# david8862/tf-keras-deeplabv3p-model-set

Hardware: AMD Instinct MI355X
Metric: images/sec (513x513, 21-class) MobileNetV2-DeepLabV3+ OS=16 training step (higher is better)
Workload: dtype f32

## Files before the change

tf-keras-deeplabv3p-model-set_amd/csrc/dwconv.hip:

```cpp
#include "bf16.h"
#include <stdlib.h>
#include <type_traits>

struct DwParams {
  const float* x; int ldx;
  const float* scale; const float* shift; int act;
  const float* w;
  float* y; int ldy;
  const float* dy; int lddy;
  float* partials;
  int N, H, W, C, Ho, Wo, stride, rate, pad_t, pad_l;
  int c4s, px, nslab, nbx, spr, th, nbands, ks, ks5;
  int uh;
  long long total;
  int flip, accumulate;
  int nt;
  int fast_rows;
  int tw;
  int lat;
  int bf16_io;
  const float* bb_z; int bb_ldz;
  const float* bb_scale; const float* bb_shift; const float* bb_mean; const float* bb_invstd; int bb_act;
  const float* fa_z; int fa_ldz;
  const float* fa_scale; const float* fa_shift; const float* fa_mean; const float* fa_invstd; const float* fa_coef; int fa_act;
  float* fa_dz; int fa_lddz;
  const float* up_x; int up_ld, up_h, up_w, up_C;
};

struct DwLerp { int lo, hi; float t; };
__device__ __forceinline__ DwLerp dw_lerp(int o, float scale, int in_size) {
  const float src = ((float)o + 0.5f) * scale - 0.5f;
  const float fl = floorf(src);
  DwLerp r;
  r.lo = max((int)fl, 0);
  r.hi = min((int)ceilf(src), in_size - 1);
  r.t = src - fl;
  return r;
}
__device__ __forceinline__ float4 dw_up_load(const float* img, int up_w, int up_ld, DwLerp ly, DwLerp lx) {
  const float4 tl = ld4(img + ((size_t)ly.lo * up_w + lx.lo) * up_ld);
  const float4 tr = ld4(img + ((size_t)ly.lo * up_w + lx.hi) * up_ld);
  const float4 bl = ld4(img + ((size_t)ly.hi * up_w + lx.lo) * up_ld);
  const float4 br = ld4(img + ((size_t)ly.hi * up_w + lx.hi) * up_ld);
  float4 o;
#define DW_LERP2(f) { const float top = tl.f + (tr.f - tl.f) * lx.t; const float bot = bl.f + (br.f - bl.f) * lx.t; o.f = top + (bot - top) * ly.t; }
  DW_LERP2(x) DW_LERP2(y) DW_LERP2(z) DW_LERP2(w)
#undef DW_LERP2
  return o;
}

__device__ __forceinline__ void bnb_accumulate(float4 (&s1)[2], float4 g, float4 zv, float4 bsc, float4 bsh, float4 bmu,
                                               float4 bis, int act) {
  const float4 u = fma4(zv, bsc, bsh);
  const float4 d = make_float4(g.x * act_grad(u.x, act), g.y * act_grad(u.y, act), g.z * act_grad(u.z, act),
                               g.w * act_grad(u.w, act));
  const float4 xh = make_float4((zv.x - bmu.x) * bis.x, (zv.y - bmu.y) * bis.y, (zv.z - bmu.z) * bis.z, (zv.w - bmu.w) * bis.w);
  s1[0] = add4(s1[0], d);
  s1[1] = fma4(d, xh, s1[1]);
}

template <int PRO>
__device__ __forceinline__ float4 prologue4(float4 v, float4 sc, float4 sh, int act) {
  if (PRO == 0) return v;
  v = fma4(v, sc, sh);
  if (PRO == 2) v = act_apply4(v, act);
  return v;
}

template <int KS, int TW, int S, int PRO, bool BNB = false, bool UP = false>
__global__ __launch_bounds__(256) void dw_fwd_seg(DwParams p) {
  constexpr int SEG = (TW - 1) * S + KS;
  const int b = blockIdx.x;
  const int slab = b / p.nbx;
  const int bx = b - slab * p.nbx;
  const int t = threadIdx.x;
  const int pl = t / p.c4s;
  const int cl = t - pl * p.c4s;
  const bool active = pl < p.px;
  const int cbase4 = slab * p.c4s;
  const int c = (cbase4 + cl) * 4;
  float4 s1[2] = {zero4(), zero4()};
  constexpr bool WLDS = KS == 5;
  extern __shared__ __attribute__((aligned(16))) float4 dw_w_lds[];
  if (WLDS) {
    for (int i = t; i < KS * KS * p.c4s; i += 256) {
      const int tap = i / p.c4s, lane = i - tap * p.c4s;
      dw_w_lds[i] = ld4(p.w + (size_t)(p.flip ? KS * KS - 1 - tap : tap) * p.C + (cbase4 + lane) * 4);
    }
    __syncthreads();
  }
  if (active) {
    float4 wreg[WLDS ? 1 : KS * KS];
    if (!WLDS) {
#pragma unroll
      for (int i = 0; i < KS * KS; ++i) wreg[i] = ld4(p.w + (size_t)(p.flip ? KS * KS - 1 - i : i) * p.C + c);
    }
    auto wtap = [&](int i) { return WLDS ? dw_w_lds[i * p.c4s + cl] : wreg[WLDS ? 0 : i]; };
    float4 sc = make_float4(1.f, 1.f, 1.f, 1.f), sh = zero4();
    if (p.scale) { sc = ld4(p.scale + c); sh = ld4(p.shift + c); }
    float4 bsc = zero4(), bsh = zero4(), bmu = zero4(), bis = zero4();
    if (BNB) { bsc = ld4(p.bb_scale + c); bsh = ld4(p.bb_shift + c); bmu = ld4(p.bb_mean + c); bis = ld4(p.bb_invstd + c); }
    const int act = p.act;
    const int th = p.th, nbands = p.nbands, rate = p.rate;
    XcdRange r = xcd_range(p.total, bx, p.nbx, p.px, pl);
    for (int s = r.begin; s < r.end; s += r.step) {
      const int strip = s % p.spr;
      int t2 = s / p.spr;
      const int band = t2 % nbands;
      t2 /= nbands;
      const int phase = t2 % (rate * rate);
      const int n = t2 / (rate * rate);
      const int py = phase / rate, pxo = phase - py * rate;
      const int u0 = strip * TW;
      const int v0 = band * p.uh / nbands, v1 = (band + 1) * p.uh / nbands;
      const int ox0 = pxo + u0 * rate;
      const int ix0 = ox0 * S - p.pad_l;
      const float* ximg = p.x + (size_t)n * p.H * p.W * p.ldx + c;
      int coff[SEG];
      bool cok[SEG];
#pragma unroll
      for (int i = 0; i < SEG; ++i) {
        const int ix = ix0 + i * rate;
        cok[i] = ix >= 0 && ix < p.W;
        coff[i] = ix * p.ldx;
      }
      DwLerp lxs[UP ? SEG : 1];
      const bool upl = UP && c < p.up_C;
      const float* uimg = nullptr;
      float usy = 0.f;
      if (UP) {
        const float usx = (float)p.up_w / (float)p.W;
        usy = (float)p.up_h / (float)p.H;
#pragma unroll
        for (int i = 0; i < SEG; ++i) lxs[i] = dw_lerp(min(max(ix0 + i * rate, 0), p.W - 1), usx, p.up_w);
        uimg = p.up_x + (size_t)n * p.up_h * p.up_w * p.up_ld + (upl ? c : 0);
      }
      float4 win[KS][SEG];
      float4 raw[S][SEG];
      {
        const int oy = py + v0 * rate;
#pragma unroll
        for (int ky = 0; ky < KS; ++ky) {
          const int iy = oy * S - p.pad_t + ky * rate;
          const bool yok = iy >= 0 && iy < p.H;
          const float* xrow = ximg + (size_t)iy * p.W * p.ldx;
#pragma unroll
          for (int i = 0; i < SEG; ++i) {
            win[ky][i] = zero4();
            if (yok && cok[i]) win[ky][i] = (UP && upl) ? dw_up_load(uimg, p.up_w, p.up_ld, dw_lerp(iy, usy, p.up_h), lxs[UP ? i : 0]) : ld4(xrow + coff[i]);
          }
        }
#pragma unroll
        for (int ky = 0; ky < KS; ++ky) {
          const int iy = oy * S - p.pad_t + ky * rate;
          const bool yok = iy >= 0 && iy < p.H;
#pragma unroll
          for (int i = 0; i < SEG; ++i) {
            const float4 a = prologue4<PRO>(win[ky][i], sc, sh, act);
            win[ky][i] = (yok && cok[i]) ? a : zero4();
          }
        }
      }
      const int vmax = (p.Ho - py + rate - 1) / rate;
      const int vend = v1 < vmax ? v1 : vmax;
      int coffc[SEG];
#pragma unroll
      for (int i = 0; i < SEG; ++i) coffc[i] = min(max(ix0 + i * rate, 0), p.W - 1) * p.ldx;
      auto row = [&](int v, auto fast_c, auto load_c) __attribute__((always_inline)) {
        constexpr bool FAST = decltype(fast_c)::value, LOAD = decltype(load_c)::value;
        const int oy = py + v * rate;
        const bool more = LOAD;
        float4 zv[TW];
        if (BNB) {
          const float* zrow = p.bb_z + (((size_t)n * p.Ho + oy) * p.Wo + ox0) * p.bb_ldz + c;
#pragma unroll
          for (int tw = 0; tw < TW; ++tw) zv[tw] = ld4(zrow + (size_t)min(tw * rate, p.Wo - 1 - ox0) * p.bb_ldz);
        }
        bool nyok[S];
#pragma unroll
        for (int q = 0; q < S; ++q) {
          const int iy = (oy + rate) * S - p.pad_t + (KS - S + q) * rate;
          nyok[q] = more && iy >= 0 && iy < p.H;
          if (FAST) {
            if (LOAD) {
              const float* xrow = ximg + (size_t)min(max(iy, 0), p.H - 1) * p.W * p.ldx;
#pragma unroll
              for (int i = 0; i < SEG; ++i) raw[q][i] = ld4(xrow + coffc[i]);
            }
          } else {
            const float* xrow = ximg + (size_t)iy * p.W * p.ldx;
#pragma unroll
            for (int i = 0; i < SEG; ++i) {
              raw[q][i] = zero4();
              if (nyok[q] && cok[i]) raw[q][i] = (UP && upl) ? dw_up_load(uimg, p.up_w, p.up_ld, dw_lerp(iy, usy, p.up_h), lxs[UP ? i : 0]) : ld4(xrow + coff[i]);
            }
          }
        }
        if (FAST) __builtin_amdgcn_sched_barrier(0);
        float4 acc[TW];
#pragma unroll
        for (int i = 0; i < TW; ++i) acc[i] = zero4();
        if (WLDS) asm volatile("" ::: "memory");
#pragma unroll
        for (int ky = 0; ky < KS; ++ky)
#pragma unroll
          for (int kx = 0; kx < KS; ++kx) {
            const float4 wv = wtap(ky * KS + kx);
#pragma unroll
            for (int tw = 0; tw < TW; ++tw) acc[tw] = fma4(win[ky][tw * S + kx], wv, acc[tw]);
          }
        float* yrow = p.y + (((size_t)n * p.Ho + oy) * p.Wo + ox0) * p.ldy + c;
#pragma unroll
        for (int tw = 0; tw < TW; ++tw) {
          if (FAST || ox0 + tw * rate < p.Wo) {
            float4 vv = acc[tw];
            float* yp = yrow + (size_t)tw * rate * p.ldy;
            if (!FAST && p.accumulate) vv = add4(vv, ld4(yp));
            if (FAST) { if (PRO != 0) st4_nt(yp, vv); else st4(yp, vv); }
            else if (p.nt) st4_nt(yp, vv); else st4(yp, vv);
            if (BNB) {
              bnb_accumulate(s1, vv, zv[tw], bsc, bsh, bmu, bis, p.bb_act);
            } else {
              s1[0] = add4(s1[0], vv);
              s1[1] = fma4(vv, vv, s1[1]);
            }
          }
        }
        if (!LOAD) return;
        if (FAST) __builtin_amdgcn_sched_barrier(0);
#pragma unroll
        for (int ky = 0; ky + S < KS; ++ky)
#pragma unroll
          for (int i = 0; i < SEG; ++i) win[ky][i] = win[ky + S][i];
#pragma unroll
        for (int q = 0; q < S; ++q)
#pragma unroll
          for (int i = 0; i < SEG; ++i) {
            float4 a = prologue4<PRO>(raw[q][i], sc, sh, act);
            if (FAST) asm volatile("" : "+v"(a.x), "+v"(a.y), "+v"(a.z), "+v"(a.w));
            win[KS - S + q][i] = (nyok[q] && cok[i]) ? a : zero4();
          }
      };
      constexpr bool HAS_FAST = PRO != 0 && !BNB && !UP;
      const bool fast = HAS_FAST && !p.accumulate && p.fast_rows && p.nt && ox0 + (TW - 1) * rate < p.Wo;
      if (HAS_FAST && fast) {
        for (int v = v0; v + 1 < vend; ++v) row(v, std::true_type{}, std::true_type{});
        if (vend > v0) row(vend - 1, std::true_type{}, std::false_type{});
      } else {
        for (int v = v0; v + 1 < vend; ++v) row(v, std::false_type{}, std::true_type{});
        if (vend > v0) row(vend - 1, std::false_type{}, std::false_type{});
      }
    }
  }
  if (p.partials) block_reduce_store<2>(s1, active, pl, cl, p.c4s, p.px, cbase4, p.C, p.partials + (size_t)bx * 2 * p.C);
}

__device__ __forceinline__ void pin4(float4& v) {
  asm volatile("" : "+v"(v.x), "+v"(v.y), "+v"(v.z), "+v"(v.w) : : "memory");
}

template <int TW, int PRO>
__global__ __launch_bounds__(256, 2) void dw5_rows(DwParams p) {
  constexpr int KS = 5, SEG = TW + KS - 1;
  const int b = blockIdx.x;
  const int slab = b / p.nbx;
  const int bx = b - slab * p.nbx;
  const int t = threadIdx.x;
  const int pl = t / p.c4s;
  const int cl = t - pl * p.c4s;
  const bool active = pl < p.px;
  const int cbase4 = slab * p.c4s;
  const int c = (cbase4 + cl) * 4;
  float4 s1[2] = {zero4(), zero4()};
  extern __shared__ __attribute__((aligned(16))) float4 dw_w_lds[];
  for (int i = t; i < KS * KS * p.c4s; i += 256) {
    const int tap = i / p.c4s, lane = i - tap * p.c4s;
    dw_w_lds[i] = ld4(p.w + (size_t)(p.flip ? KS * KS - 1 - tap : tap) * p.C + (cbase4 + lane) * 4);
  }
  __syncthreads();
  if (active) {
    float4 sc = make_float4(1.f, 1.f, 1.f, 1.f), sh = zero4();
    if (p.scale) { sc = ld4(p.scale + c); sh = ld4(p.shift + c); }
    const int act = p.act;
    const int th = p.th, nbands = p.nbands, rate = p.rate;
    const float4* wl = dw_w_lds + cl;
    const int c4s = p.c4s;
    XcdRange r = xcd_range(p.total, bx, p.nbx, p.px, pl);
    for (int s = r.begin; s < r.end; s += r.step) {
      const int strip = s % p.spr;
      int t2 = s / p.spr;
      const int band = t2 % nbands;
      t2 /= nbands;
      const int phase = t2 % (rate * rate);
      const int n = t2 / (rate * rate);
      const int py = phase / rate, pxo = phase - py * rate;
      const int v0 = band * p.uh / nbands, v1 = (band + 1) * p.uh / nbands;
      const int oy0 = py + v0 * rate;
      if (oy0 >= p.Ho) continue;
      int nv = (p.Ho - oy0 + rate - 1) / rate;
      if (nv > v1 - v0) nv = v1 - v0;
      const int ox0 = pxo + strip * TW * rate;
      const int ix0 = ox0 - p.pad_l;
      const float* ximg = p.x + (size_t)n * p.H * p.W * p.ldx + c;
      int coff[SEG];
      bool cok[SEG];
#pragma unroll
      for (int i = 0; i < SEG; ++i) {
        const int ix = ix0 + i * rate;
        cok[i] = ix >= 0 && ix < p.W;
        coff[i] = ix * p.ldx;
      }
      const int iy0 = oy0 - p.pad_t;
      const int nj = nv + KS - 1;
      float4 acc[KS][TW];
#pragma unroll
      for (int q = 0; q < KS; ++q)
#pragma unroll
        for (int tw = 0; tw < TW; ++tw) acc[q][tw] = zero4();
      float4 a[SEG];
      {
        const bool yok = iy0 >= 0 && iy0 < p.H;
        const float* xrow = ximg + (size_t)iy0 * p.W * p.ldx;
#pragma unroll
        for (int i = 0; i < SEG; ++i) {
          a[i] = zero4();
          if (yok && cok[i]) a[i] = ld4(xrow + coff[i]);
        }
#pragma unroll
        for (int i = 0; i < SEG; ++i) {
          const float4 v = prologue4<PRO>(a[i], sc, sh, act);
          a[i] = (yok && cok[i]) ? v : zero4();
        }
      }
      for (int j = 0; j < nj; ++j) {
        float4 nxt[SEG];
        const int iyn = iy0 + (j + 1) * rate;
        const bool nyok = j + 1 < nj && iyn >= 0 && iyn < p.H;
        {
          const float* xrow = ximg + (size_t)iyn * p.W * p.ldx;
#pragma unroll
          for (int i = 0; i < SEG; ++i) {
            nxt[i] = zero4();
            if (nyok && cok[i]) nxt[i] = ld4(xrow + coff[i]);
          }
        }
        const int vdone = j - (KS - 1);
        const int oyd = oy0 + vdone * rate;
        asm volatile("" ::: "memory");
        float4 wrow[2][KS];
#pragma unroll
        for (int kx = 0; kx < KS; ++kx) wrow[0][kx] = wl[kx * c4s];
#pragma unroll
        for (int ky = 0; ky < KS; ++ky) {
          if (ky + 1 < KS) {
#pragma unroll
            for (int kx = 0; kx < KS; ++kx) wrow[(ky + 1) & 1][kx] = wl[((ky + 1) * KS + kx) * c4s];
          }
#pragma unroll
          for (int kx = 0; kx < KS; ++kx) {
#pragma unroll
            for (int tw = 0; tw < TW; ++tw)
              acc[KS - 1 - ky][tw] = fma4(a[tw + kx], wrow[ky & 1][kx], acc[KS - 1 - ky][tw]);
          }
#pragma unroll
          for (int tw = 0; tw < TW; ++tw) pin4(acc[KS - 1 - ky][tw]);
        }
        if (vdone >= 0) {
          float* yrow = p.y + (((size_t)n * p.Ho + oyd) * p.Wo + ox0) * p.ldy + c;
#pragma unroll
          for (int tw = 0; tw < TW; ++tw) {
            if (ox0 + tw * rate < p.Wo) {
              float4 vv = acc[0][tw];
              float* yp = yrow + (size_t)tw * rate * p.ldy;
              if (p.accumulate) vv = add4(vv, ld4(yp));
              if (p.nt) st4_nt(yp, vv); else st4(yp, vv);
              s1[0] = add4(s1[0], vv);
              s1[1] = fma4(vv, vv, s1[1]);
            }
          }
        }
#pragma unroll
        for (int q = 0; q + 1 < KS; ++q)
#pragma unroll
          for (int tw = 0; tw < TW; ++tw) acc[q][tw] = acc[q + 1][tw];
#pragma unroll
        for (int tw = 0; tw < TW; ++tw) acc[KS - 1][tw] = zero4();
#pragma unroll
        for (int i = 0; i < SEG; ++i) {
          const float4 v = prologue4<PRO>(nxt[i], sc, sh, act);
          a[i] = (nyok && cok[i]) ? v : zero4();
        }
      }
    }
  }
  if (p.partials) block_reduce_store<2>(s1, active, pl, cl, p.c4s, p.px, cbase4, p.C, p.partials + (size_t)bx * 2 * p.C);
}

template <int TW, int PRO>
__global__ __launch_bounds__(256, 2) void dw5_wgrad_rows(DwParams p) {
  constexpr int KS = 5, SEG = TW + KS - 1;
  const int b = blockIdx.x;
  const int slab = b / p.nbx;
  const int bx = b - slab * p.nbx;
  const int t = threadIdx.x;
  const int pl = t / p.c4s;
  const int cl = t - pl * p.c4s;
  const bool active = pl < p.px;
  const int cbase4 = slab * p.c4s;
  const int c = (cbase4 + cl) * 4;
  float4 wacc[KS * KS];
#pragma unroll
  for (int i = 0; i < KS * KS; ++i) wacc[i] = zero4();
  if (active) {
    float4 sc = make_float4(1.f, 1.f, 1.f, 1.f), sh = zero4();
    if (p.scale) { sc = ld4(p.scale + c); sh = ld4(p.shift + c); }
    const int act = p.act;
    const int nbands = p.nbands, rate = p.rate;
    XcdRange r = xcd_range(p.total, bx, p.nbx, p.px, pl);
    for (int s = r.begin; s < r.end; s += r.step) {
      const int strip = s % p.spr;
      int t2 = s / p.spr;
      const int band = t2 % nbands;
      t2 /= nbands;
      const int phase = t2 % (rate * rate);
      const int n = t2 / (rate * rate);
      const int py = phase / rate, pxo = phase - py * rate;
      const int v0 = band * p.uh / nbands, v1 = (band + 1) * p.uh / nbands;
      const int oy0 = py + v0 * rate;
      if (oy0 >= p.Ho) continue;
      int nv = (p.Ho - oy0 + rate - 1) / rate;
      if (nv > v1 - v0) nv = v1 - v0;
      const int ox0 = pxo + strip * TW * rate;
      const int ix0 = ox0 - p.pad_l;
      const float* ximg = p.x + (size_t)n * p.H * p.W * p.ldx + c;
      const float* dimg = p.dy + ((size_t)n * p.Ho * p.Wo + ox0) * p.lddy + c;
      int coff[SEG];
      bool cok[SEG];
#pragma unroll
      for (int i = 0; i < SEG; ++i) {
        const int ix = ix0 + i * rate;
        cok[i] = ix >= 0 && ix < p.W;
        coff[i] = ix * p.ldx;
      }
      bool dok[TW];
#pragma unroll
      for (int tw = 0; tw < TW; ++tw) dok[tw] = ox0 + tw * rate < p.Wo;
      const int iy0 = oy0 - p.pad_t;
      const int nj = nv + KS - 1;
      float4 a[SEG];
      float4 dyw[KS][TW];
#pragma unroll
      for (int d = 0; d < KS; ++d)
#pragma unroll
        for (int tw = 0; tw < TW; ++tw) dyw[d][tw] = zero4();
      {
        const bool yok = iy0 >= 0 && iy0 < p.H;
        const float* xrow = ximg + (size_t)iy0 * p.W * p.ldx;
#pragma unroll
        for (int i = 0; i < SEG; ++i) {
          a[i] = zero4();
          if (yok && cok[i]) a[i] = ld4(xrow + coff[i]);
        }
        const float* drow = dimg + (size_t)oy0 * p.Wo * p.lddy;
#pragma unroll
        for (int tw = 0; tw < TW; ++tw)
          if (dok[tw]) dyw[KS - 1][tw] = ld4(drow + (size_t)tw * rate * p.lddy);
#pragma unroll
        for (int i = 0; i < SEG; ++i) {
          const float4 v = prologue4<PRO>(a[i], sc, sh, act);
          a[i] = (yok && cok[i]) ? v : zero4();
        }
      }
      for (int j = 0; j < nj; ++j) {
        float4 nxt[SEG], dyn[TW];
        const int iyn = iy0 + (j + 1) * rate;
        const bool nyok = j + 1 < nj && iyn >= 0 && iyn < p.H;
        const bool dyok = j + 1 < nv;
        {
          const float* xrow = ximg + (size_t)iyn * p.W * p.ldx;
#pragma unroll
          for (int i = 0; i < SEG; ++i) {
            nxt[i] = zero4();
            if (nyok && cok[i]) nxt[i] = ld4(xrow + coff[i]);
          }
          const float* drow = dimg + (size_t)(oy0 + (j + 1) * rate) * p.Wo * p.lddy;
#pragma unroll
          for (int tw = 0; tw < TW; ++tw) {
            dyn[tw] = zero4();
            if (dyok && dok[tw]) dyn[tw] = ld4(drow + (size_t)tw * rate * p.lddy);
          }
        }
#pragma unroll
        for (int ky = 0; ky < KS; ++ky)
#pragma unroll
          for (int kx = 0; kx < KS; ++kx)
#pragma unroll
            for (int tw = 0; tw < TW; ++tw)
              wacc[ky * KS + kx] = fma4(a[tw + kx], dyw[KS - 1 - ky][tw], wacc[ky * KS + kx]);
#pragma unroll
        for (int d = 0; d + 1 < KS; ++d)
#pragma unroll
          for (int tw = 0; tw < TW; ++tw) dyw[d][tw] = dyw[d + 1][tw];
#pragma unroll
        for (int tw = 0; tw < TW; ++tw) dyw[KS - 1][tw] = dyn[tw];
#pragma unroll
        for (int i = 0; i < SEG; ++i) {
          const float4 v = prologue4<PRO>(nxt[i], sc, sh, act);
          a[i] = (nyok && cok[i]) ? v : zero4();
        }
      }
    }
  }
  block_reduce_store<KS * KS>(wacc, active, pl, cl, p.c4s, p.px, cbase4, p.C,
                              p.partials + (size_t)bx * KS * KS * p.C);
}

template <int KS, int TW, int S, int PRO, bool BNA = false, bool UP = false>
__global__ __launch_bounds__(256) void dw_bwd_weight_seg(DwParams p) {
  constexpr int SEG = (TW - 1) * S + KS;
  const int b = blockIdx.x;
  const int slab = b / p.nbx;
  const int bx = b - slab * p.nbx;
  const int t = threadIdx.x;
  const int pl = t / p.c4s;
  const int cl = t - pl * p.c4s;
  const bool active = pl < p.px;
  const int cbase4 = slab * p.c4s;
  const int c = (cbase4 + cl) * 4;
  float4 wacc[KS * KS];
#pragma unroll
  for (int i = 0; i < KS * KS; ++i) wacc[i] = zero4();
  if (active) {
    float4 sc = make_float4(1.f, 1.f, 1.f, 1.f), sh = zero4();
    if (p.scale) { sc = ld4(p.scale + c); sh = ld4(p.shift + c); }
    const int act = p.act;
    const int th = p.th, nbands = p.nbands, rate = p.rate;
    float4 bA = zero4(), bC = zero4(), bD = zero4(), bsc = make_float4(1.f, 1.f, 1.f, 1.f), bsh = zero4();
    if (BNA) {
      if (p.fa_scale) { bsc = ld4(p.fa_scale + c); bsh = ld4(p.fa_shift + c); }
      const float4 mu = ld4(p.fa_mean + c), is = ld4(p.fa_invstd + c);
      const float4 c0 = ld4(p.fa_coef + c), c1 = ld4(p.fa_coef + p.C + c), c2 = ld4(p.fa_coef + 2 * p.C + c);
      bA = c0;
      bC = mul4(mul4(c0, is), c2);
      bD = make_float4(bC.x * mu.x - c0.x * c1.x, bC.y * mu.y - c0.y * c1.y, bC.z * mu.z - c0.z * c1.z, bC.w * mu.w - c0.w * c1.w);
    }
    XcdRange r = xcd_range(p.total, bx, p.nbx, p.px, pl);
    for (int s = r.begin; s < r.end; s += r.step) {
      const int strip = s % p.spr;
      int t2 = s / p.spr;
      const int band = t2 % nbands;
      t2 /= nbands;
      const int phase = t2 % (rate * rate);
      const int n = t2 / (rate * rate);
      const int py = phase / rate, pxo = phase - py * rate;
      const int u0 = strip * TW;
      const int v0 = band * p.uh / nbands, v1 = (band + 1) * p.uh / nbands;
      const int ox0 = pxo + u0 * rate;
      const int ix0 = ox0 * S - p.pad_l;
      const float* ximg = p.x + (size_t)n * p.H * p.W * p.ldx + c;
      int coff[SEG];
      bool cok[SEG];
#pragma unroll
      for (int i = 0; i < SEG; ++i) {
        const int ix = ix0 + i * rate;
        cok[i] = ix >= 0 && ix < p.W;
        coff[i] = ix * p.ldx;
      }
      DwLerp lxs[UP ? SEG : 1];
      const bool upl = UP && c < p.up_C;
      const float* uimg = nullptr;
      float usy = 0.f;
      if (UP) {
        const float usx = (float)p.up_w / (float)p.W;
        usy = (float)p.up_h / (float)p.H;
#pragma unroll
        for (int i = 0; i < SEG; ++i) lxs[i] = dw_lerp(min(max(ix0 + i * rate, 0), p.W - 1), usx, p.up_w);
        uimg = p.up_x + (size_t)n * p.up_h * p.up_w * p.up_ld + (upl ? c : 0);
      }
      float4 win[KS][SEG];
      float4 raw[S][SEG];
      {
        const int oy = py + v0 * rate;
#pragma unroll
        for (int ky = 0; ky < KS; ++ky) {
          const int iy = oy * S - p.pad_t + ky * rate;
          const bool yok = iy >= 0 && iy < p.H;
          const float* xrow = ximg + (size_t)iy * p.W * p.ldx;
#pragma unroll
          for (int i = 0; i < SEG; ++i) {
            win[ky][i] = zero4();
            if (yok && cok[i]) win[ky][i] = (UP && upl) ? dw_up_load(uimg, p.up_w, p.up_ld, dw_lerp(iy, usy, p.up_h), lxs[UP ? i : 0]) : ld4(xrow + coff[i]);
          }
        }
#pragma unroll
        for (int ky = 0; ky < KS; ++ky) {
          const int iy = oy * S - p.pad_t + ky * rate;
          const bool yok = iy >= 0 && iy < p.H;
#pragma unroll
          for (int i = 0; i < SEG; ++i) {
            const float4 a = prologue4<PRO>(win[ky][i], sc, sh, act);
            win[ky][i] = (yok && cok[i]) ? a : zero4();
          }
        }
      }
      for (int v = v0; v < v1; ++v) {
        const int oy = py + v * rate;
        if (oy >= p.Ho) break;
        const bool more = v + 1 < v1 && oy + rate < p.Ho;
        bool nyok[S];
#pragma unroll
        for (int q = 0; q < S; ++q) {
          const int iy = (oy + rate) * S - p.pad_t + (KS - S + q) * rate;
          nyok[q] = more && iy >= 0 && iy < p.H;
          const float* xrow = ximg + (size_t)iy * p.W * p.ldx;
#pragma unroll
          for (int i = 0; i < SEG; ++i) {
            raw[q][i] = zero4();
            if (nyok[q] && cok[i]) raw[q][i] = (UP && upl) ? dw_up_load(uimg, p.up_w, p.up_ld, dw_lerp(iy, usy, p.up_h), lxs[UP ? i : 0]) : ld4(xrow + coff[i]);
          }
        }
        float4 dyv[TW];
        const float* drow = p.dy + (((size_t)n * p.Ho + oy) * p.Wo + ox0) * p.lddy + c;
#pragma unroll
        for (int tw = 0; tw < TW; ++tw) {
          dyv[tw] = zero4();
          if (ox0 + tw * rate < p.Wo) dyv[tw] = ld4(drow + (size_t)tw * rate * p.lddy);
        }
        if (BNA) {
          const size_t pix = ((size_t)n * p.Ho + oy) * p.Wo + ox0;
          const float* zrow = p.fa_z + pix * p.fa_ldz + c;
          float4 zv[TW];
#pragma unroll
          for (int tw = 0; tw < TW; ++tw) {
            zv[tw] = zero4();
            if (ox0 + tw * rate < p.Wo) zv[tw] = ld4(zrow + (size_t)tw * rate * p.fa_ldz);
          }
          const int fact = p.fa_act;
#pragma unroll
          for (int tw = 0; tw < TW; ++tw) {
            const float4 z = zv[tw], g = dyv[tw];
            const float4 u = fma4(z, bsc, bsh);
            const float4 v = make_float4(fmaf(bA.x, g.x * act_grad(u.x, fact), fmaf(-bC.x, z.x, bD.x)),
                                         fmaf(bA.y, g.y * act_grad(u.y, fact), fmaf(-bC.y, z.y, bD.y)),
                                         fmaf(bA.z, g.z * act_grad(u.z, fact), fmaf(-bC.z, z.z, bD.z)),
                                         fmaf(bA.w, g.w * act_grad(u.w, fact), fmaf(-bC.w, z.w, bD.w)));
            const bool ok = ox0 + tw * rate < p.Wo;
            if (ok && p.fa_dz) st4(p.fa_dz + (pix + (size_t)tw * rate) * p.fa_lddz + c, v);
            dyv[tw] = ok ? v : zero4();
          }
        }
#pragma unroll
        for (int ky = 0; ky < KS; ++ky)
#pragma unroll
          for (int kx = 0; kx < KS; ++kx)
#pragma unroll
            for (int tw = 0; tw < TW; ++tw) wacc[ky * KS + kx] = fma4(win[ky][tw * S + kx], dyv[tw], wacc[ky * KS + kx]);
#pragma unroll
        for (int ky = 0; ky + S < KS; ++ky)
#pragma unroll
          for (int i = 0; i < SEG; ++i) win[ky][i] = win[ky + S][i];
#pragma unroll
        for (int q = 0; q < S; ++q)
#pragma unroll
          for (int i = 0; i < SEG; ++i) {
            const float4 a = prologue4<PRO>(raw[q][i], sc, sh, act);
            win[KS - S + q][i] = (nyok[q] && cok[i]) ? a : zero4();
          }
      }
    }
  }
  block_reduce_store<KS * KS>(wacc, active, pl, cl, p.c4s, p.px, cbase4, p.C,
// ... 402 lines not shown
  const int pl = t / p.c4s;
  const int cl = t - pl * p.c4s;
  const bool active = pl < p.px;
  const int cbase4 = slab * p.c4s;
  const int c = (cbase4 + cl) * 4;
  float4 wacc[KS * KS];
#pragma unroll
  for (int i = 0; i < KS * KS; ++i) wacc[i] = zero4();
  if (active) {
    float4 sc = make_float4(1.f, 1.f, 1.f, 1.f), sh = zero4();
    if (p.scale) { sc = ld4(p.scale + c); sh = ld4(p.shift + c); }
    const int act = p.act;
    XcdRange r = xcd_range(p.total, bx, p.nbx, p.px, pl);
    for (int s = r.begin; s < r.end; s += r.step) {
      const int ox = s % p.Wo;
      const int row = s / p.Wo;
      const int oy = row % p.Ho;
      const int n = row / p.Ho;
      const float4 g = ld4(p.dy + (((size_t)n * p.Ho + oy) * p.Wo + ox) * p.lddy + c);
      const float* ximg = p.x + (size_t)n * p.H * p.W * p.ldx + c;
      float4 v[KS * KS];
      bool ok[KS * KS];
#pragma unroll
      for (int ky = 0; ky < KS; ++ky) {
        const int iy = oy * p.stride - p.pad_t + ky * p.rate;
        const bool yok = iy >= 0 && iy < p.H;
#pragma unroll
        for (int kx = 0; kx < KS; ++kx) {
          const int ix = ox * p.stride - p.pad_l + kx * p.rate;
          const bool o = yok && ix >= 0 && ix < p.W;
          ok[ky * KS + kx] = o;
          v[ky * KS + kx] = zero4();
          if (o) v[ky * KS + kx] = ld4(ximg + ((size_t)iy * p.W + ix) * p.ldx);
        }
      }
#pragma unroll
      for (int i = 0; i < KS * KS; ++i) {
        const float4 a = prologue4<PRO>(v[i], sc, sh, act);
        if (ok[i]) wacc[i] = fma4(a, g, wacc[i]);
      }
    }
  }
  block_reduce_store<KS * KS>(wacc, active, pl, cl, p.c4s, p.px, cbase4, p.C,
                              p.partials + (size_t)bx * KS * KS * p.C);
}

static int check_dw_common(const char* fn, const void* x, int ldx, int C, int k) {
  DL3P_CHECK_ARG(C > 0 && C % 4 == 0, "%s: C=%d must be a positive multiple of 4", fn, C);
  DL3P_CHECK_ARG(ldx % 4 == 0 && ldx >= C, "%s: ld=%d must be a multiple of 4 and >= C", fn, ldx);
  DL3P_CHECK_ARG(aligned16(x), "%s: tensor pointer must be 16-byte aligned", fn);
  DL3P_CHECK_ARG(k == 3 || k == 5, "%s: kernel size %d unsupported (3 or 5)", fn, k);
  return DL3P_OK;
}

static int pick_band(long long items_per_row_band, int rows, int px, int nslab) {
  static const int want_env = getenv("DL3P_DW_WANT") ? atoi(getenv("DL3P_DW_WANT")) : DL3P_NUM_CUS * 3 / 2;
  const long long want = want_env;
  static const int force = getenv("DL3P_DW_BAND") ? atoi(getenv("DL3P_DW_BAND")) : 0;
  if (force && rows <= 40) return force;
  int th = 16;
  while (th > 1 && (items_per_row_band * ceil_div(rows, th) / px) * nslab < want) th >>= 1;
  return th;
}

static int dw5_rows_tw(int uw) {
  static const int v = getenv("DL3P_DW5_ROWS") ? atoi(getenv("DL3P_DW5_ROWS")) : -1;
  if (v >= 0) return v;
  return uw <= 40 ? 4 : 2;
}
static int dw5_tw(int uw) { return dw5_rows_tw(uw) == 4 ? 4 : 2; }

struct DwTuned { int role, N, H, W, C, k, stride, rate, per_cu, want, maxth, tw; };
#include "dw_tuned.h"
int dl3p_dw_force_per_cu = 0, dl3p_dw_force_want = 0, dl3p_dw_force_maxth = 0, dl3p_dw_force_tw = 0, dl3p_dw_use_table = -1;
static const DwTuned* dw_tuned_lookup(const DwParams& p) {
  if (dl3p_dw_use_table < 0) dl3p_dw_use_table = getenv("DL3P_DW_TUNED") ? atoi(getenv("DL3P_DW_TUNED")) : 1;
  if (!dl3p_dw_use_table) return nullptr;
  const int role = p.bb_z ? 2 : (p.flip ? 1 : (p.dy ? 3 : 0));
  for (size_t i = 0; i < sizeof(g_dw_tuned) / sizeof(g_dw_tuned[0]); ++i) {
    const DwTuned& e = g_dw_tuned[i];
    if (e.role == role && e.N == p.N && e.H == p.H && e.W == p.W && e.C == p.C && e.k == (p.ks5 ? 5 : 3) && e.stride == p.stride &&
        e.rate == p.rate)
      return &e;
  }
  return nullptr;
}

static int fwd_plan(DwParams& p, int per_cu = 8, bool window5 = false, int tw5 = 0) {
  int kind = 0;
  int t_want = 0, t_maxth = 0, t_tw = 0;
  if (const DwTuned* e = dw_tuned_lookup(p)) {
    if (e->per_cu) per_cu = e->per_cu;
    t_want = e->want; t_maxth = e->maxth; t_tw = e->tw;
  }
  if (dl3p_dw_force_tw) t_tw = dl3p_dw_force_tw;
  if (dl3p_dw_force_per_cu) per_cu = dl3p_dw_force_per_cu;
  if (dl3p_dw_force_want) t_want = dl3p_dw_force_want;
  if (dl3p_dw_force_maxth) t_maxth = dl3p_dw_force_maxth;
  if (p.ks5 && !window5) kind = 0;
  else if (p.stride == 1 && ceil_div(p.Wo, p.rate) >= 4) kind = 1;
  else if (p.stride == 2 && p.rate == 1 && p.Wo >= 4) kind = 2;
  if (kind == 0 && p.ks == 3 && p.stride == 1 && p.pad_t == p.rate && p.pad_l == p.rate && p.Ho == p.H && p.Wo == p.W &&
      2 * p.rate >= p.H && 2 * p.rate >= p.W && p.rate < p.H && p.rate < p.W &&
      (long long)p.N * p.H * p.W * (p.ldx > p.ldy ? p.ldx : p.ldy) < (1LL << 31)) { kind = 3; p.lat = 2; }
  static const int lat3 = getenv("DL3P_DW_LAT3") ? atoi(getenv("DL3P_DW_LAT3")) : 1;
  if (kind == 0 && lat3 && p.ks == 3 && p.stride == 1 && p.pad_t == p.rate && p.pad_l == p.rate && p.Ho == p.H && p.Wo == p.W &&
      3 * p.rate >= p.H && 3 * p.rate >= p.W && p.rate < p.H && p.rate < p.W &&
      (long long)p.N * p.H * p.W * (p.ldx > p.ldy ? p.ldx : p.ldy) < (1LL << 31)) { kind = 3; p.lat = 3; }
  if (kind == 3) {
    p.spr = p.rate; p.th = 1; p.nbands = p.rate;
    p.total = (long long)p.N * p.rate * p.rate;
  } else if (kind == 0) {
    p.spr = p.Wo; p.th = 1; p.nbands = p.Ho;
    p.total = (long long)p.N * p.Ho * p.Wo;
  } else {
    const int r = p.rate;
    const int uw = ceil_div(p.Wo, r), uh = ceil_div(p.Ho, r);
    const int TW = p.ks5 ? (kind == 1 ? (tw5 ? tw5 : dw5_tw(uw)) : 1) : (kind == 1 ? (t_tw == 2 ? 2 : 4) : 2);
    p.tw = TW;
    p.spr = ceil_div(uw, TW);
    static const int balance = getenv("DL3P_DW_BALANCE") ? atoi(getenv("DL3P_DW_BALANCE")) : 2;
    if (balance == 2) {
      static const int want_env = getenv("DL3P_DW_WANT") ? atoi(getenv("DL3P_DW_WANT")) : DL3P_NUM_CUS * 3 / 2;
      static const int maxth_env = getenv("DL3P_DW_MAXTH") ? atoi(getenv("DL3P_DW_MAXTH")) : 16;
      const int want = t_want ? t_want : want_env, maxth = t_maxth ? t_maxth : maxth_env;
      const long long per_band = (long long)p.N * r * r * p.spr;
      int nb = ceil_div(uh, maxth);
      while (nb < uh && (per_band * nb / p.px) * p.nslab < want) ++nb;
      p.nbands = nb;
      p.th = ceil_div(uh, nb);
      p.uh = uh;
    } else {
      p.th = pick_band((long long)p.N * r * r * p.spr, uh, p.px, p.nslab);
      if (p.th > uh) p.th = uh;
      p.nbands = ceil_div(uh, p.th);
      p.uh = balance ? uh : p.nbands * p.th;
    }
    p.total = (long long)p.N * r * r * p.nbands * p.spr;
  }
  static const int lat2_per_cu = getenv("DL3P_LAT2_PER_CU") ? atoi(getenv("DL3P_LAT2_PER_CU")) : DL3P_LAT2_PER_CU;
  static const int lat3_per_cu = getenv("DL3P_LAT3_PER_CU") ? atoi(getenv("DL3P_LAT3_PER_CU")) : 3;
  p.nbx = pick_nbx(p.total, p.px, p.nslab, kind == 3 ? (p.lat == 3 ? lat3_per_cu : lat2_per_cu) : per_cu);
  return kind;
}

template <int KS, int PRO>
static void launch_fwd_pro(const DwParams& p, int kind, dim3 grid, hipStream_t st) {
  dim3 block(256);
  if (KS == 5) {
    const size_t lds = (size_t)25 * p.c4s * sizeof(float4);
    const int rows_tw = dw5_rows_tw(ceil_div(p.Wo, p.rate));
    if (kind == 1 && rows_tw == 4) dl3p_launch(dw5_rows<4, PRO>, grid, block, lds, st, p);
    else if (kind == 1 && rows_tw == 2) dl3p_launch(dw5_rows<2, PRO>, grid, block, lds, st, p);
    else if (kind == 1) dl3p_launch(dw_fwd_seg<5, 2, 1, PRO>, grid, block, lds, st, p);
    else if (kind == 2) dl3p_launch(dw_fwd_seg<5, 1, 2, PRO>, grid, block, lds, st, p);
    else dl3p_launch(dw_fwd_gather<5, PRO>, grid, block, 0, st, p);
    return;
  }
  if (p.up_x) {
    if constexpr (PRO == 2) {
      if (p.tw == 2) dl3p_launch(dw_fwd_seg<3, 2, 1, 2, false, true>, grid, block, 0, st, p);
      else dl3p_launch(dw_fwd_seg<3, 4, 1, 2, false, true>, grid, block, 0, st, p);
    }
    return;
  }
  if (kind == 1 && p.tw == 2) dl3p_launch(dw_fwd_seg<3, 2, 1, PRO>, grid, block, 0, st, p);
  else if (kind == 1) dl3p_launch(dw_fwd_seg<3, 4, 1, PRO>, grid, block, 0, st, p);
  else if (kind == 2) dl3p_launch(dw_fwd_seg<3, 2, 2, PRO>, grid, block, 0, st, p);
  else if (kind == 3 && p.lat == 3) dl3p_launch(dw_fwd_lattice3<PRO>, grid, block, 0, st, p);
  else if (kind == 3) dl3p_launch(dw_fwd_lattice2<PRO>, grid, block, 0, st, p);
  else dl3p_launch(dw_fwd_gather<3, PRO>, grid, block, 0, st, p);
}

static int plan_forward(DwParams& p, int KS, int tw5) {
  p.ks = KS;
  p.ks5 = KS == 5;
  static const int dwf_per_cu = getenv("DL3P_DWF_PER_CU") ? atoi(getenv("DL3P_DWF_PER_CU")) : 8;
  if (KS == 5) {
    const int c4 = p.C / 4;
    int best = 1;
    for (int d = 1; d <= c4 && d <= 64; ++d)
      if (c4 % d == 0 && (256 / d) * d >= (256 / best) * best) best = d;
    p.c4s = best; p.px = 256 / best; p.nslab = c4 / best;
  }
  return fwd_plan(p, dwf_per_cu, true, tw5);
}

template <int KS>
static void launch_fwd(const DwParams& p0, hipStream_t st) {
  DwParams p = p0;
  const int kind = plan_forward(p, KS, 0);
  static const int nt_mask = getenv("DL3P_DW_NT") ? atoi(getenv("DL3P_DW_NT")) : 3;
  p.nt = (p.flip == 0 && !p.accumulate) ? ((kind == 0 ? (nt_mask >> 1) : nt_mask) & 1) : 0;
  static const int fast_rows = getenv("DL3P_DW_FAST_ROWS") ? atoi(getenv("DL3P_DW_FAST_ROWS")) : 1;
  const long long out_bytes = (long long)p.N * p.Ho * p.Wo * p.C * 4;
  p.fast_rows = fast_rows >= 2 || (fast_rows == 1 && p.nt && out_bytes >= (200ll << 20));
  dim3 grid(p.nbx * p.nslab);
  const int pro = (p.act != DL3P_ACT_NONE) ? 2 : (p.scale ? 1 : 0);
  if (pro == 2) launch_fwd_pro<KS, 2>(p, kind, grid, st);
  else if (pro == 1) launch_fwd_pro<KS, 1>(p, kind, grid, st);
  else launch_fwd_pro<KS, 0>(p, kind, grid, st);
}

static thread_local DwParams t_dw_up = {};
extern "C" int dl3p_dw_upsampled_input(const float* up_x, int up_ld, int up_h, int up_w, int up_C, void* stream) {
  (void)stream;
  DL3P_CHECK_ARG(up_x && aligned16(up_x) && up_ld % 4 == 0 && up_C > 0 && up_C % 4 == 0 && up_ld >= up_C && up_h > 0 && up_w > 0,
                 "dl3p_dw_upsampled_input: bad arguments");
  t_dw_up.up_x = up_x; t_dw_up.up_ld = up_ld; t_dw_up.up_h = up_h; t_dw_up.up_w = up_w; t_dw_up.up_C = up_C;
  return DL3P_OK;
}
static int plan_forward(DwParams& p, int KS, int tw5);
static int dwconv2d_bwd_weight_impl(const float* x, int ldx, const float* in_scale, const float* in_shift, int in_act, const float* dy,
                                    int lddy, float* gw, float* workspace, size_t workspace_bytes, int N, int H, int W, int C, int k,
                                    int stride, int rate, int pad_t, int pad_l, int Ho, int Wo, int* rows_out, void* stream,
                                    const DwParams* fold, int* kind_out);
extern "C" int dl3p_dw_upsampled_input_supported(int role, int N, int H, int W, int C, int up_C, int k, int stride, int rate, int pad_t,
                                                 int pad_l, int Ho, int Wo) {
  if (k != 3 || stride != 1 || rate != 1 || C <= 0 || C % 4 || up_C <= 0 || up_C % 4 || up_C > C || N <= 0 || H <= 0 || W <= 0) return 0;
  DwParams p = {};
  p.N = N; p.H = H; p.W = W; p.C = C; p.Ho = Ho; p.Wo = Wo; p.stride = stride; p.rate = rate; p.pad_t = pad_t; p.pad_l = pad_l;
  if (role == 0) {
    pick_lanes(C, &p.c4s, &p.px, &p.nslab);
    return plan_forward(p, 3, 0) == 1;
  }
  int kind = -1;
  alignas(16) static float dummy[4];
  const int rc = dwconv2d_bwd_weight_impl(dummy, C, nullptr, nullptr, DL3P_ACT_NONE, dummy, C, dummy, dummy, (size_t)-1, N, H, W, C, k,
                                          stride, rate, pad_t, pad_l, Ho, Wo, nullptr, nullptr, nullptr, &kind);
  return rc == DL3P_OK && kind == 1;
}
static bool dw_take_up(DwParams& p) {
  if (!t_dw_up.up_x) return false;
  p.up_x = t_dw_up.up_x; p.up_ld = t_dw_up.up_ld; p.up_h = t_dw_up.up_h; p.up_w = t_dw_up.up_w; p.up_C = t_dw_up.up_C;
  t_dw_up.up_x = nullptr;
  return true;
}

extern "C" int dl3p_dwconv2d_fwd(const float* x, int ldx, const float* in_scale, const float* in_shift, int in_act,
                                 const float* w, float* y, int ldy, float* stat_partials, int* rows_out,
                                 int N, int H, int W, int C, int k, int stride, int rate, int pad_t, int pad_l,
                                 int Ho, int Wo, void* stream) {
  int rc = check_dw_common("dl3p_dwconv2d_fwd", x, ldx, C, k);
  if (rc) return rc;
  DL3P_CHECK_ARG(x && w && y, "dl3p_dwconv2d_fwd: null pointer");
  DL3P_CHECK_ARG(ldy % 4 == 0 && ldy >= C && aligned16(y) && aligned16(w), "dl3p_dwconv2d_fwd: bad y/w layout");
  DL3P_CHECK_ARG(N > 0 && H > 0 && W > 0 && Ho > 0 && Wo > 0 && stride >= 1 && rate >= 1, "dl3p_dwconv2d_fwd: bad dims");
  DwParams p = {};
  p.x = x; p.ldx = ldx; p.scale = in_scale; p.shift = in_shift; p.act = in_act; p.w = w;
  p.y = y; p.ldy = ldy; p.partials = stat_partials;
  p.N = N; p.H = H; p.W = W; p.C = C; p.Ho = Ho; p.Wo = Wo; p.stride = stride; p.rate = rate;
  p.pad_t = pad_t; p.pad_l = pad_l;
  pick_lanes(C, &p.c4s, &p.px, &p.nslab);
  const bool up = dw_take_up(p);
  {
    DwParams q = p;
    const int kind = plan_forward(q, k, 0);
    if (rows_out) *rows_out = q.nbx;
    DL3P_CHECK_ARG(!up || (k == 3 && stride == 1 && rate == 1 && kind == 1 && in_scale && in_act != DL3P_ACT_NONE && p.up_C <= C),
                   "dl3p_dwconv2d_fwd: the upsampled-input form serves 3x3 stride-1 window launches behind a BatchNorm + activation (dl3p_dw_upsampled_input_supported)");
  }
  hipStream_t st = (hipStream_t)stream;
  if (k == 3) launch_fwd<3>(p, st); else launch_fwd<5>(p, st);
  DL3P_CHECK_LAUNCH("dl3p_dwconv2d_fwd");
  return DL3P_OK;
}

extern "C" int dl3p_dwconv2d_bwd_data(const float* dy, int lddy, const float* w, float* gx, int ldgx, int accumulate,
                                      int N, int H, int W, int C, int k, int stride, int rate, int pad_t, int pad_l,
                                      int Ho, int Wo, void* stream) {
  int rc = check_dw_common("dl3p_dwconv2d_bwd_data", dy, lddy, C, k);
  if (rc) return rc;
  DL3P_CHECK_ARG(dy && w && gx, "dl3p_dwconv2d_bwd_data: null pointer");
  DL3P_CHECK_ARG(ldgx % 4 == 0 && ldgx >= C && aligned16(gx) && aligned16(w), "dl3p_dwconv2d_bwd_data: bad gx/w layout");
  hipStream_t st = (hipStream_t)stream;
  DwParams p = {};
  p.w = w; p.C = C; p.N = N; p.accumulate = accumulate;
  pick_lanes(C, &p.c4s, &p.px, &p.nslab);
  if (stride == 1) {
    p.x = dy; p.ldx = lddy; p.y = gx; p.ldy = ldgx; p.flip = 1;
    p.H = Ho; p.W = Wo; p.Ho = H; p.Wo = W; p.stride = 1; p.rate = rate;
    p.pad_t = rate * (k - 1) - pad_t; p.pad_l = rate * (k - 1) - pad_l;
    p.act = DL3P_ACT_NONE;
    if (k == 3) launch_fwd<3>(p, st); else launch_fwd<5>(p, st);
  } else {
    p.dy = dy; p.lddy = lddy; p.y = gx; p.ldy = ldgx;
    p.H = H; p.W = W; p.Ho = Ho; p.Wo = Wo; p.stride = stride; p.rate = rate; p.pad_t = pad_t; p.pad_l = pad_l;
    if (stride == 2 && rate == 1) {
      p.th = ((H - 1 + pad_t) >> 1) + 1;
      p.spr = ((W - 1 + pad_l) >> 1) + 1;
      p.total = (long long)N * p.th * p.spr;
      p.nbx = pick_nbx(p.total, p.px, p.nslab);
      dim3 grid(p.nbx * p.nslab), block(256);
      if (k == 3) hipLaunchKernelGGL((dw_bwd_data_s2<3>), grid, block, 0, st, p);
      else hipLaunchKernelGGL((dw_bwd_data_s2<5>), grid, block, 0, st, p);
    } else {
      p.total = (long long)N * H * W;
      p.nbx = pick_nbx(p.total, p.px, p.nslab);
      dim3 grid(p.nbx * p.nslab), block(256);
      if (k == 3) hipLaunchKernelGGL((dw_bwd_data_strided<3>), grid, block, 0, st, p);
      else hipLaunchKernelGGL((dw_bwd_data_strided<5>), grid, block, 0, st, p);
    }
  }
  DL3P_CHECK_LAUNCH("dl3p_dwconv2d_bwd_data");
  return DL3P_OK;
}

extern "C" int dl3p_bn_bwd_reduce(const float* g, int ldg, const float* z, int ldz, const float* scale, const float* shift,
                                  int act, const float* save_mean, const float* save_invstd, float* partials,
                                  int* rows_out, int M, int C, void* stream);
extern "C" int dl3p_dwconv2d_bwd_data_bn(const float* dy, int lddy, const float* w, float* gx, int ldgx, int accumulate,
                                         int N, int H, int W, int C, int k, int stride, int rate, int pad_t, int pad_l,
                                         int Ho, int Wo, const float* z, int ldz, const float* scale, const float* shift,
                                         int act, const float* save_mean, const float* save_invstd, float* partials,
                                         int* rows_out, void* stream) {
  int rc = check_dw_common("dl3p_dwconv2d_bwd_data_bn", dy, lddy, C, k);
  if (rc) return rc;
// ... 299 lines not shown
```

Measured before the change: 1354.

## Split depthwise forward fast-row path into separate kernel instantiation and raise occupancy bounds

Moves the fast-row path of the segmented depthwise forward kernel into its own template instantiation (FAST_K), chosen on the host, so the general kernel no longer carries both code paths and their register pressure. The general path becomes a simple row loop. It also adds a min-blocks-per-CU launch bound of 2 for the 5x5 stride-2 activation forward kernel and for the BN-backward weight-gradient kernel, to raise occupancy. The tighter bounds risk register spills, and the extra instantiations add compile time and code size.

```diff
diff --git a/tf-keras-deeplabv3p-model-set_amd/csrc/dwconv.hip b/tf-keras-deeplabv3p-model-set_amd/csrc/dwconv.hip
--- a/tf-keras-deeplabv3p-model-set_amd/csrc/dwconv.hip
+++ b/tf-keras-deeplabv3p-model-set_amd/csrc/dwconv.hip
@@ -67,8 +67,9 @@
   return v;
 }
 
-template <int KS, int TW, int S, int PRO, bool BNB = false, bool UP = false>
-__global__ __launch_bounds__(256) void dw_fwd_seg(DwParams p) {
+template <int KS, int TW, int S, int PRO, bool BNB = false, bool UP = false, bool FAST_K = false>
+__global__ __launch_bounds__(256, (KS == 5 && S == 2 && PRO == 2 && !FAST_K) ? 2 : 1) void dw_fwd_seg(DwParams p) {
+  static_assert(!FAST_K || (PRO != 0 && !BNB && !UP), "counted-wait rows: forward launches only");
   constexpr int SEG = (TW - 1) * S + KS;
   const int b = blockIdx.x;
   const int slab = b / p.nbx;
@@ -161,15 +162,72 @@
           }
         }
       }
-      const int vmax = (p.Ho - py + rate - 1) / rate;
-      const int vend = v1 < vmax ? v1 : vmax;
-      int coffc[SEG];
-#pragma unroll
-      for (int i = 0; i < SEG; ++i) coffc[i] = min(max(ix0 + i * rate, 0), p.W - 1) * p.ldx;
-      auto row = [&](int v, auto fast_c, auto load_c) __attribute__((always_inline)) {
-        constexpr bool FAST = decltype(fast_c)::value, LOAD = decltype(load_c)::value;
+      if constexpr (FAST_K) {
+        if (ox0 + (TW - 1) * rate < p.Wo) {
+          int coffc[SEG];
+#pragma unroll
+          for (int i = 0; i < SEG; ++i) coffc[i] = min(max(ix0 + i * rate, 0), p.W - 1) * p.ldx;
+          auto row = [&](int v, auto load_c) __attribute__((always_inline)) {
+            constexpr bool LOAD = decltype(load_c)::value;
+            const int oy = py + v * rate;
+            bool nyok[S];
+#pragma unroll
+            for (int q = 0; q < S; ++q) {
+              const int iy = (oy + rate) * S - p.pad_t + (KS - S + q) * rate;
+              nyok[q] = LOAD && iy >= 0 && iy < p.H;
+              if (LOAD) {
+                const float* xrow = ximg + (size_t)min(max(iy, 0), p.H - 1) * p.W * p.ldx;
+#pragma unroll
+                for (int i = 0; i < SEG; ++i) raw[q][i] = ld4(xrow + coffc[i]);
+              }
+            }
+            __builtin_amdgcn_sched_barrier(0);
+            float4 acc[TW];
+#pragma unroll
+            for (int i = 0; i < TW; ++i) acc[i] = zero4();
+            if (WLDS) asm volatile("" ::: "memory");
+#pragma unroll
+            for (int ky = 0; ky < KS; ++ky)
+#pragma unroll
+              for (int kx = 0; kx < KS; ++kx) {
+                const float4 wv = wtap(ky * KS + kx);
+#pragma unroll
+                for (int tw = 0; tw < TW; ++tw) acc[tw] = fma4(win[ky][tw * S + kx], wv, acc[tw]);
+              }
+            float* yrow = p.y + (((size_t)n * p.Ho + oy) * p.Wo + ox0) * p.ldy + c;
+#pragma unroll
+            for (int tw = 0; tw < TW; ++tw) {
+              const float4 vv = acc[tw];
+              st4_nt(yrow + (size_t)tw * rate * p.ldy, vv);
+              s1[0] = add4(s1[0], vv);
+              s1[1] = fma4(vv, vv, s1[1]);
+            }
+            if (!LOAD) return;
+            __builtin_amdgcn_sched_barrier(0);
+#pragma unroll
+            for (int ky = 0; ky + S < KS; ++ky)
+#pragma unroll
+              for (int i = 0; i < SEG; ++i) win[ky][i] = win[ky + S][i];
+#pragma unroll
+            for (int q = 0; q < S; ++q)
+#pragma unroll
+              for (int i = 0; i < SEG; ++i) {
+                float4 a = prologue4<PRO>(raw[q][i], sc, sh, act);
+                asm volatile("" : "+v"(a.x), "+v"(a.y), "+v"(a.z), "+v"(a.w));
+                win[KS - S + q][i] = (nyok[q] && cok[i]) ? a : zero4();
+              }
+          };
+          const int vmax = (p.Ho - py + rate - 1) / rate;
+          const int vend = v1 < vmax ? v1 : vmax;
+          for (int v = v0; v + 1 < vend; ++v) row(v, std::true_type{});
+          if (vend > v0) row(vend - 1, std::false_type{});
+          continue;
+        }
+      }
+      for (int v = v0; v < v1; ++v) {
         const int oy = py + v * rate;
-        const bool more = LOAD;
+        if (oy >= p.Ho) break;
+        const bool more = v + 1 < v1 && oy + rate < p.Ho;
         float4 zv[TW];
         if (BNB) {
           const float* zrow = p.bb_z + (((size_t)n * p.Ho + oy) * p.Wo + ox0) * p.bb_ldz + c;
@@ -181,22 +239,13 @@
         for (int q = 0; q < S; ++q) {
           const int iy = (oy + rate) * S - p.pad_t + (KS - S + q) * rate;
           nyok[q] = more && iy >= 0 && iy < p.H;
-          if (FAST) {
-            if (LOAD) {
-              const float* xrow = ximg + (size_t)min(max(iy, 0), p.H - 1) * p.W * p.ldx;
-#pragma unroll
-              for (int i = 0; i < SEG; ++i) raw[q][i] = ld4(xrow + coffc[i]);
-            }
-          } else {
-            const float* xrow = ximg + (size_t)iy * p.W * p.ldx;
-#pragma unroll
-            for (int i = 0; i < SEG; ++i) {
-              raw[q][i] = zero4();
-              if (nyok[q] && cok[i]) raw[q][i] = (UP && upl) ? dw_up_load(uimg, p.up_w, p.up_ld, dw_lerp(iy, usy, p.up_h), lxs[UP ? i : 0]) : ld4(xrow + coff[i]);
-            }
-          }
-        }
-        if (FAST) __builtin_amdgcn_sched_barrier(0);
+          const float* xrow = ximg + (size_t)iy * p.W * p.ldx;
+#pragma unroll
+          for (int i = 0; i < SEG; ++i) {
+            raw[q][i] = zero4();
+            if (nyok[q] && cok[i]) raw[q][i] = (UP && upl) ? dw_up_load(uimg, p.up_w, p.up_ld, dw_lerp(iy, usy, p.up_h), lxs[UP ? i : 0]) : ld4(xrow + coff[i]);
+          }
+        }
         float4 acc[TW];
 #pragma unroll
         for (int i = 0; i < TW; ++i) acc[i] = zero4();
@@ -212,12 +261,11 @@
         float* yrow = p.y + (((size_t)n * p.Ho + oy) * p.Wo + ox0) * p.ldy + c;
 #pragma unroll
         for (int tw = 0; tw < TW; ++tw) {
-          if (FAST || ox0 + tw * rate < p.Wo) {
+          if (ox0 + tw * rate < p.Wo) {
             float4 vv = acc[tw];
             float* yp = yrow + (size_t)tw * rate * p.ldy;
-            if (!FAST && p.accumulate) vv = add4(vv, ld4(yp));
-            if (FAST) { if (PRO != 0) st4_nt(yp, vv); else st4(yp, vv); }
-            else if (p.nt) st4_nt(yp, vv); else st4(yp, vv);
+            if (p.accumulate) vv = add4(vv, ld4(yp));
+            if (p.nt) st4_nt(yp, vv); else st4(yp, vv);
             if (BNB) {
               bnb_accumulate(s1, vv, zv[tw], bsc, bsh, bmu, bis, p.bb_act);
             } else {
@@ -226,8 +274,6 @@
             }
           }
         }
-        if (!LOAD) return;
-        if (FAST) __builtin_amdgcn_sched_barrier(0);
 #pragma unroll
         for (int ky = 0; ky + S < KS; ++ky)
 #pragma unroll
@@ -236,19 +282,9 @@
         for (int q = 0; q < S; ++q)
 #pragma unroll
           for (int i = 0; i < SEG; ++i) {
-            float4 a = prologue4<PRO>(raw[q][i], sc, sh, act);
-            if (FAST) asm volatile("" : "+v"(a.x), "+v"(a.y), "+v"(a.z), "+v"(a.w));
+            const float4 a = prologue4<PRO>(raw[q][i], sc, sh, act);
             win[KS - S + q][i] = (nyok[q] && cok[i]) ? a : zero4();
           }
-      };
-      constexpr bool HAS_FAST = PRO != 0 && !BNB && !UP;
-      const bool fast = HAS_FAST && !p.accumulate && p.fast_rows && p.nt && ox0 + (TW - 1) * rate < p.Wo;
-      if (HAS_FAST && fast) {
-        for (int v = v0; v + 1 < vend; ++v) row(v, std::true_type{}, std::true_type{});
-        if (vend > v0) row(vend - 1, std::true_type{}, std::false_type{});
-      } else {
-        for (int v = v0; v + 1 < vend; ++v) row(v, std::false_type{}, std::true_type{});
-        if (vend > v0) row(vend - 1, std::false_type{}, std::false_type{});
       }
     }
   }
@@ -516,7 +552,7 @@
 }
 
 template <int KS, int TW, int S, int PRO, bool BNA = false, bool UP = false>
-__global__ __launch_bounds__(256) void dw_bwd_weight_seg(DwParams p) {
+__global__ __launch_bounds__(256, (BNA && !UP) ? 2 : 1) void dw_bwd_weight_seg(DwParams p) {
   constexpr int SEG = (TW - 1) * S + KS;
   const int b = blockIdx.x;
   const int slab = b / p.nbx;
@@ -1225,8 +1261,15 @@
     const int rows_tw = dw5_rows_tw(ceil_div(p.Wo, p.rate));
     if (kind == 1 && rows_tw == 4) dl3p_launch(dw5_rows<4, PRO>, grid, block, lds, st, p);
     else if (kind == 1 && rows_tw == 2) dl3p_launch(dw5_rows<2, PRO>, grid, block, lds, st, p);
-    else if (kind == 1) dl3p_launch(dw_fwd_seg<5, 2, 1, PRO>, grid, block, lds, st, p);
-    else if (kind == 2) dl3p_launch(dw_fwd_seg<5, 1, 2, PRO>, grid, block, lds, st, p);
+    else if (kind == 1 || kind == 2) {
+      const bool fast = PRO != 0 && p.fast_rows && p.nt && !p.accumulate;
+      if constexpr (PRO != 0) {
+        if (fast && kind == 1) dl3p_launch(dw_fwd_seg<5, 2, 1, PRO, false, false, true>, grid, block, lds, st, p);
+        else if (fast) dl3p_launch(dw_fwd_seg<5, 1, 2, PRO, false, false, true>, grid, block, lds, st, p);
+      }
+      if (!fast && kind == 1) dl3p_launch(dw_fwd_seg<5, 2, 1, PRO>, grid, block, lds, st, p);
+      else if (!fast) dl3p_launch(dw_fwd_seg<5, 1, 2, PRO>, grid, block, lds, st, p);
+    }
     else dl3p_launch(dw_fwd_gather<5, PRO>, grid, block, 0, st, p);
     return;
   }
@@ -1236,6 +1279,14 @@
       else dl3p_launch(dw_fwd_seg<3, 4, 1, 2, false, true>, grid, block, 0, st, p);
     }
     return;
+  }
+  if constexpr (PRO != 0) {
+    if (p.fast_rows && p.nt && !p.accumulate && (kind == 1 || kind == 2)) {
+      if (kind == 1 && p.tw == 2) dl3p_launch(dw_fwd_seg<3, 2, 1, PRO, false, false, true>, grid, block, 0, st, p);
+      else if (kind == 1) dl3p_launch(dw_fwd_seg<3, 4, 1, PRO, false, false, true>, grid, block, 0, st, p);
+      else dl3p_launch(dw_fwd_seg<3, 2, 2, PRO, false, false, true>, grid, block, 0, st, p);
+      return;
+    }
   }
   if (kind == 1 && p.tw == 2) dl3p_launch(dw_fwd_seg<3, 2, 1, PRO>, grid, block, 0, st, p);
   else if (kind == 1) dl3p_launch(dw_fwd_seg<3, 4, 1, PRO>, grid, block, 0, st, p);
```

Measured after the change: 1368 (median of 6 runs). 1.01x the previous value.
